# exosports/transit

Hardware: AMD Instinct MI355X
Metric: wavenumber-points*layers/sec (CH4 2-4um emission spectrum) (higher is better)
Workload: dtype f64; 1 GPU; BASELINE configs[1]: CH4-demo-shaped emission: 2500-5000 cm-1 @1 cm-1, wnosamp 2160, CH4 lines, eclipse, 5 angles, H2-H2 CIA; n_wn=2501, n_layers=100, layers_needed=81, n_lines=1000000, parallelism=one GPU

## Files before the change

transit_amd/csrc/hip/trx_api.hip:

```cpp
#include <hip/hip_runtime.h>
#include <rccl/rccl.h>
#include <dlfcn.h>

#include <algorithm>
#include <chrono>
#include <cmath>
#include <cstdio>
#include <cstdlib>
#include <cstring>
#include <atomic>
#include <condition_variable>
#include <initializer_list>
#include <memory>
#include <mutex>
#include <string>
#include <thread>
#include <vector>

#include "transit_hip.h"
#include "trx_kernels.hip.h"
#include "trx_walk.hip.h"
#include "trx_rows.hip.h"
#include "trx_tail.hip.h"
#include "trx_lanes.hip.h"
// ... 33 lines not shown
#include "../trx_launch.h"
#include "../trx_hpdata.h"

using namespace trx;

#include "trx_handle.hip.h"

namespace {

void read_switches(Switches &w)
{
  auto set = [](const char *name) { return std::getenv(name) != nullptr; };
  auto num = [](const char *name, long long otherwise) { const char *e = std::getenv(name); return e ? std::atoll(e) : otherwise; };
  auto clamped = [&](const char *name, int lo, int hi, int otherwise) { return (int)std::max<long long>(lo, std::min<long long>(hi, num(name, otherwise))); };
  w.no_row_copy = set("TRX_NO_ROW_COPY");
  w.no_rows32 = set("TRX_NO_ROWS32");
  w.row_staging = !set("TRX_NO_ROW_STAGING");
  w.row_m8_from = num("TRX_ROWS_M8_FROM", w.row_m8_from);
  w.packed_walk = !set("TRX_NO_PACKED_WALK");
  w.packed_max_layers = clamped("TRX_PACKED_MAX_LAYERS", 1, 32, w.packed_max_layers);
  w.xcd_map = (int)num("TRX_XCD_MAP", w.xcd_map);
  w.no_binrec = set("TRX_NO_BINREC");
  const long long lanes = num("TRX_LANES_WALK", 1);
  w.lanes_walk = lanes != 0; w.lanes_force = lanes == 2;
  w.lanes_parts_most = clamped("TRX_LANES_PARTS", 2, 4, w.lanes_parts_most);
  w.ray_tail = num("TRX_RAY_TAIL", 1) != 0;
  w.cia_sums = num("TRX_CIA_SUMS", 1) != 0;
  w.cia_segments = num("TRX_CIA_SEGMENTS", 1) != 0;
  w.cia_window = num("TRX_CIA_WINDOW", 1) != 0;
  w.two_queues = num("TRX_TWO_QUEUES", 1) != 0;
  w.tail_direct = num("TRX_TAIL_DIRECT", 1) != 0;
  w.range_reach = num("TRX_RANGE_REACH", 1) != 0;
  w.shard_frames = num("TRX_SHARD_FRAMES", 1) != 0;
}

struct TableBuild { TablePlan P; DevBuf d_jobs; };

template <class F>
void for_job_batches(const std::vector<ProfileJob> &jobs, F fn)
{
  for (size_t j0 = 0; j0 < jobs.size(); j0 += 32768) fn(j0, (int)std::min<size_t>(32768, jobs.size() - j0));
}

int plan_into_handle(trx_handle *h, const trx_static *s, TableBuild &B)
{
  const char *text = "";
  const TablePlanError pe = plan_table(*s, B.P, &text);
  if (pe != kTablePlanOk) return fail(h, pe == kTablePlanArg ? TRX_E_ARG : TRX_E_UNSUPPORTED, text);
  h->adop = B.P.adop; h->alor = B.P.alor; h->psize = B.P.psize; h->poff = B.P.poff; h->tab_n = B.P.tab_n;
  h->psizeT = std::move(B.P.psizeT); h->psize_mono = B.P.psize_mono;
  if (!index_steps(h->adop.data(), s->ndop, h->dopthr)) return fail(h, TRX_E_ARG, "Doppler-width grid is not strictly increasing");
  if (!index_steps(h->alor.data(), s->nlor, h->lorthr)) h->lorthr.clear();
  return TRX_OK;
}

int upload_table_inputs(trx_handle *h, const trx_static *s, TableBuild &B)
{
  int rc;
  double coef[64]; long double fact = 1.0L;
  for (int n = 0; n < 64; n++) { if (n > 0) fact *= (long double)n; coef[n] = (double)(1.0L / (fact * (long double)(2 * n + 1))); }
  HIPCHK(h, hipMemcpyToSymbolAsync(HIP_SYMBOL(c_voigt_coef), coef, sizeof(coef), 0, hipMemcpyHostToDevice, h->stream));
  if ((rc = upload(h, B.d_jobs, B.P.jobs))) return rc;
  const size_t tab_alloc = table_alloc_floats(h->tab_n, s->osamp);
  if ((rc = ensure(h, h->d_tab, sizeof(float) * tab_alloc))) return rc;
  HIPCHK(h, hipMemsetAsync(h->d_tab.p, 0, sizeof(float) * tab_alloc, h->stream));
  h->tab = h->d_tab.as<float>() + kTabPad;
// ... 514 lines not shown

struct LayerHost {
  size_t nli = 0, extra_off = 0;
  std::vector<double> &f64; std::vector<int32_t> &i32;
  const int32_t *psmax = nullptr;
  LayerHost(std::vector<double> &f, std::vector<int32_t> &i) : f64(f), i32(i) {}
};

inline double layer_negct(double temp) { return -kExpCte * kTliEfct / temp; }
inline double layer_strength(const trx_handle *h, int i, double z) { return kSigCte * h->iso_ratio[i] / (h->iso_mass[i] * z); }

inline int dop_index(const trx_handle *h, double v, int from)
{
  const double *thr = h->dopthr.data();
  while (from + 1 < h->ndop && v >= thr[from + 1]) from++;
  while (v < thr[from]) from--;
  return from;
}
inline int lor_index(const trx_handle *h, double v, int from)
{
  if (h->lorthr.empty()) return nearest_index(h->alor.data(), v, 0, h->nlor);
  const double *thr = h->lorthr.data();
  while (from + 1 < h->nlor && v >= thr[from + 1]) from++;
  while (v < thr[from]) from--;
  return from;
}
inline int dop_index_far(const trx_handle *h, double v)
{
  const double *thr = h->dopthr.data();
  return (int)(std::upper_bound(thr + 1, thr + h->ndop, v) - thr) - 1;
}

int prep_layers(trx_handle *h, int nr, const double *temp_k, const double *density ,
                const double *zpart , size_t extra_doubles, LayerHost &LH)
{
  const int niso = h->niso, nmol = h->nmol;
  const size_t nli = (size_t)nr * std::max(niso, 1);
  LH.nli = nli; LH.extra_off = 7 * nli;
  LH.f64.assign(7 * nli + extra_doubles, 0.0);
  LH.i32.assign(4 * nli, 0);
  double *negct = &LH.f64[0], *strength = negct + nr, *dens = strength + nli, *alphad = dens + nli,
         *alphal = alphad + nli, *wcut = alphal + nli;
  int32_t *idop0 = &LH.i32[0], *ilor = idop0 + nli, *psmax = ilor + nli, *npre = psmax + nli;
  LH.psmax = psmax;
  h->dens_over_m.resize(nmol);
  double *dm = h->dens_over_m.data();
  h->guess_dop.assign((size_t)std::max(niso, 1), 0); h->guess_lor.assign((size_t)std::max(niso, 1), 0);
  h->guess_a0.assign((size_t)std::max(niso, 1), 0); h->guess_a1.assign((size_t)std::max(niso, 1), 0); h->guess_npre.assign((size_t)std::max(niso, 1), -1);
  for (int r = 0; r < nr; r++) {
    const double temp = temp_k[r];
    if (!(temp > 0)) return fail(h, TRX_E_ARG, "non-positive layer temperature");
    negct[r] = layer_negct(temp);
    const double fdoppler = std::sqrt(2 * kKb * temp / kAmu) * kSqrtLn2 / kLs;
    const double florentz = std::sqrt(2 * kKb * temp / kPi / kAmu) / (kAmu * kLs);
    for (int j = 0; j < nmol; j++) dm[j] = density[(size_t)j * nr + r] / h->mol_mass[j];
    for (int i = 0; i < niso; i++) {
      double al = 0.0;
      const double *csd_i = &h->pair_csd[(size_t)i * nmol], *sq_i = &h->pair_sqrt[(size_t)i * nmol];
      for (int j = 0; j < nmol; j++)
        al += dm[j] * csd_i[j] * csd_i[j] * sq_i[j];
      al *= florentz;
      const double ad = fdoppler / h->iso_sqrtm[i];
      const size_t k = (size_t)r * niso + i;
      alphal[k] = al; alphad[k] = ad;
      idop0[k] = h->guess_dop[i] = dop_index(h, ad * h->wn_i, h->guess_dop[i]);
      ilor[k]  = h->guess_lor[i] = lor_index(h, al, h->guess_lor[i]);
      strength[k] = layer_strength(h, i, zpart[(size_t)i * nr + r]);
      dens[k] = density[(size_t)h->iso_imol[i] * nr + r];
      wcut[k] = doppler_refresh_cut(ad, al);
      const bool has_lines = h->iso_wmax[i] > 0;
      const int a0 = has_lines ? (h->guess_a0[i] = dop_index(h, ad * h->iso_wmin[i], h->guess_a0[i])) : idop0[k];
      const int a1 = has_lines ? (h->guess_a1[i] = dop_index(h, ad * h->iso_wmax[i], h->guess_a1[i])) : idop0[k];
      const int32_t *psl = &h->psizeT[(size_t)ilor[k] * h->ndop];
      auto widest_of = [&](int i0, int i1) {
        if (i0 > i1) std::swap(i0, i1);
        if (h->psize_mono) return psl[i1];
        int32_t m = 0;
        for (int d = i0; d <= i1; d++) m = std::max(m, psl[d]);
        return m;
      };
      int32_t pm = widest_of(std::min(idop0[k], std::min(a0, a1)), std::max(idop0[k], std::max(a0, a1)));
      if (h->sw.shard_frames && has_lines) {
// ... 441 lines not shown
}

static int run_check(trx_handle *h, const trx_atm *a, const trx_opts *o)
{
  const int nr = a->nlayer;
  if (nr < 3) return fail(h, TRX_E_ARG, "at least three layers are needed");
  if (!h->saved.empty() && (int)h->saved.size() != nr) return fail(h, TRX_E_ARG, "restored extinction has another number of layers");
  if (!h->saved.empty() && h->has_grid) return fail(h, TRX_E_UNSUPPORTED, "restored extinction together with an opacity grid");
  if (o->solution != TRX_SOL_ECLIPSE && o->solution != TRX_SOL_TRANSIT) return fail(h, TRX_E_ARG, "unknown solution");
  if (o->solution == TRX_SOL_ECLIPSE && (o->nangles < 1 || o->nangles > kMaxAngles || !o->angles_deg))
    return fail(h, TRX_E_ARG, "eclipse needs 1..16 angles");
  if (o->solution == TRX_SOL_TRANSIT && o->modlevel != 1 && o->modlevel != -1) return fail(h, TRX_E_UNSUPPORTED, "modlevel must be 1 or -1");
  if (!(o->ethresh > 0)) return fail(h, TRX_E_ARG, "ethresh must be positive");
  if ((o->cloud_flag >= 2 || o->scat_flag == 2) && !a->abund && o->cloud_flag >= 2) return fail(h, TRX_E_ARG, "cloud model needs abundances");
  for (int i = 1; i < nr; i++) if (!(a->radius[i] > a->radius[i-1])) return fail(h, TRX_E_ARG, "radii must ascend");
  return TRX_OK;
}

namespace {

constexpr ScheduleCaps kScheduleCaps{kEmisRowsAbove, kTailRays, kTailSteps, 65536, kMaxChunk, kTauH};
static_assert(kTailSteps == 2, "the side-queue tail waits for ev_walk1 alone: the main queue may carry exactly one walk ahead of it");

struct Run {
  trx_handle *const h; const trx_atm *const a; const trx_opts *const o;
  double *const spectrum; void *const d_spectrum; trx_debug *const dbg; const Products want;
  const std::chrono::steady_clock::time_point t_host0;

  const int nr = a->nlayer; const int64_t nsh = h->nsh; const hipStream_t st = h->stream;
  const bool eager = o->eager != 0, prof = o->profile != 0, count = o->profile >= 2;
  const bool vertical = o->solution == TRX_SOL_ECLIPSE, extras_on = o->scat_flag != 0 || o->cloud_flag != 0;
  const bool pipelined = !h->has_grid;
  const bool stop_at_hint_ok = !h->has_grid && !eager && h->hint_layers > 0 && h->hint_layers <= nr;
  const bool stage_spec = spectrum && !d_spectrum && nsh <= (1 << 20);

  LayerHost LH{h->run_f64, h->run_i32};
  int gstride = 0; size_t mw_doubles = 0, n_geom_all = 0, nli = 0, n_f64 = 0, n_geom = 0, n_ip = 0, n_cd = 0, n_i32 = 0;
  size_t off_geom = 0, off_ip = 0, off_cd = 0, off_i32 = 0, in_bytes = 0;

  const bool ride_along = nsh <= 65536;
  bool early_front = false; double *kmax_run = nullptr; RunInit RI{};

  LayerDev Y{}; const double *d_wcut = nullptr; const int32_t *d_npre = nullptr;
  const double *d_press = nullptr, *d_tempk = nullptr, *d_mdens = nullptr, *d_nH = nullptr, *d_scatpol = nullptr, *d_rad = nullptr;
  const double *d_gw = nullptr, *d_gh0 = nullptr, *d_mw = nullptr, *d_mh0 = nullptr, *d_pw = nullptr, *d_ipv = nullptr, *d_ciadens = nullptr;
  double *d_out = nullptr; PlanInput P{};

  hipStream_t tst = nullptr;
  hipStream_t queue(Queue q) const { return q == kQMain ? st : q == kQSide ? h->stream4 : h->stream2; }
  hipEvent_t event(const QueueOp &op) const {
    switch (op.ev) {
      case kEvInputs: return h->ev_inputs; case kEvCia: return h->ev_cia; case kEvJoin: return h->ev_join; case kEvWalk1: return h->ev_walk1;
      case kEvStepDone: return h->ev_ac[(size_t)op.idx]; case kEvRecordsFree: return h->ev_cb[(size_t)op.idx];
      default: return nullptr;
    }
  }

  TailChoice tail;
  TailArgs TA{}; int tail_nct = 0;
  const size_t tail_blocks = (size_t)((nsh + kTailRays - 1) / kTailRays);

  int r_top = nr - 1; bool resumed = false;
  ScheduleState sched;
  CombineArgs comb[2];
  std::vector<uint8_t> layer_walked;

  int flags[8] = {}, status[4] = {}; double ms_cia = 0;
  std::vector<unsigned long long> counters;
  Spans spans; Spans *const sp = prof ? &spans : nullptr;
  std::chrono::steady_clock::time_point t_host_prep = t_host0, t_host_queued = t_host0, t_lap = t_host0;
  const bool lap_on = log_sink().fn && log_sink().max_level >= TRX_LOG_DEBUG; std::string laps;

  bool in_flight = false;
  ~Run() { if (in_flight) { (void)hipStreamSynchronize(h->stream4); (void)hipStreamSynchronize(h->stream2); (void)hipStreamSynchronize(h->stream); } }

  void lap(const char *what) {
    if (!lap_on) return;
    const auto n = std::chrono::steady_clock::now();
    char b[64]; std::snprintf(b, sizeof b, " %s %.0f", what, 1e3 * std::chrono::duration<double, std::milli>(n - t_lap).count());
    laps += b; t_lap = n;
  }
  void model_args(TauArgs &T) const; void tau_args(TauArgs &T, int r_top_, int nc_) const; void emis_args(EmisArgs &E) const; void mod_args(ModArgs &M) const;
  void launch_tau(const TauArgs &T, hipStream_t q) const; void launch_ray_tail() const;
  void launch_run_init() const
  { hipLaunchKernelGGL(k_run_init, dim3((unsigned)std::min<long long>((std::max<long long>(nsh, 3LL * nr) + 255) / 256, 65536)), dim3(256), 0, st, RI); }
  int layout(); int front_maxima(); void host_inputs();
  int workspaces(); int front_inputs(); int grid_weights();
  int plan_first_pass(); int pass(); int resume(); int finish();
  int issue(const QueueOp &op); SweepMode sweep_mode(const QueueOp &op) const;
  int walk(const QueueOp &op); int grid_step(const PlanStep &s); int cia_group(); int restore_rows(const QueueOp &op); int tau_substep(const QueueOp &op);
  int spectrum_kernel(); int ray_tail();
  int results(const PassEnd &end);
  int product_kernels();
};

void Run::model_args(TauArgs &T) const
{
  T.nr = nr; T.nsh = nsh; T.lo = h->lo; T.wn_i = h->wn_i; T.wn_d = h->wn_d; T.wn_fct = o->wn_fct;
  T.scat_flag = o->scat_flag; T.cloud_flag = o->cloud_flag; T.nmol = h->nmol;
  T.scat_pref = std::pow(10.0, o->scat_logext) * kE0H2;
  T.press = d_press; T.temp = d_tempk; T.scat_pol = d_scatpol;
  T.cloud_top = o->cloud_top; T.cloud_bot = o->cloud_bot; T.cloud_ext = o->cloud_ext; T.cloud_gamma = o->cloud_gamma;
  T.cloud_Q = o->cloud_Q; T.cloud_r = o->cloud_r; T.cloud_sig = o->cloud_sig; T.cloud_refwn = o->cloud_refwn;
  T.mdens = d_mdens; T.nH = d_nH;
  if (extras_on) { T.xf_scat = h->d_xf.as<double>(); T.xf_cloud = T.xf_scat + nsh; T.xf_const = T.xf_cloud + nsh; }
}

void Run::tau_args(TauArgs &T, int r_top_, int nc_) const
{
  T.solution = o->solution; T.rad_fct = a->rad_fct; T.toomuch = o->toomuch;
  T.r_top = r_top_; T.nc = nc_; T.rad = d_rad; T.e = h->d_e.as<double>(); T.ecs = h->d_ecs.as<double>();
  T.er = h->d_er.as<double>(); T.tau = h->d_tau.as<double>(); T.last = h->d_last.as<int>();
  T.er_all = (dbg != nullptr || eager) ? 1 : 0;
  T.gw = d_gw; T.gstride = gstride; T.gh0 = d_gh0;
  model_args(T);
  T.flags = h->d_flags.as<int>(); T.eager = eager;
  T.pw = d_pw; T.acc = h->d_acc.as<double>(); T.lay = vertical ? d_pw + 6 * (size_t)nr : nullptr;
  T.hrs = d_pw + 4 * (size_t)nr; T.hr0 = T.hrs + nr; T.status = h->d_status.as<int>();
}

void Run::emis_args(EmisArgs &E) const
// ... 50 lines not shown
  n_f64 = 7 * nli + 8 * (size_t)nr; n_geom = vertical ? n_geom_all : 1; n_ip = (size_t)nr; n_cd = (size_t)nr * h->cia.size(); n_i32 = 4 * nli;
  off_geom = n_f64; off_ip = off_geom + n_geom; off_cd = off_ip + n_ip; off_i32 = off_cd + n_cd;
  in_bytes = (8 * off_i32 + 4 * n_i32 + 8 + 15) & ~(size_t)15;
  if ((rc = ensure_pinned(h, h->h_in, in_bytes)) || (rc = ensure(h, h->d_in, in_bytes)) || (rc = ensure_small(h, nr)) ||
      (rc = ensure(h, h->d_last, sizeof(int) * nsh)) || (rc = ensure(h, h->d_acc, sizeof(double) * 2 * nsh)) ||
      (rc = ensure(h, h->d_sticky, sizeof(int) * nli)))
    return rc;
  const size_t had = h->d_kmax.bytes;
  if ((rc = ensure(h, h->d_kmax, sizeof(double) * 2 * (size_t)nr))) return rc;
  if (h->d_kmax.bytes != had || !h->kmax_clean || h->kmax_nr != nr) {
    HIPCHK(h, hipMemsetAsync(h->d_kmax.p, 0, sizeof(double) * 2 * (size_t)nr, st));
    h->kmax_parity = 0; h->kmax_nr = nr;
  }
  h->kmax_clean = false;
  kmax_run = h->d_kmax.as<double>() + (size_t)h->kmax_parity * nr;
  RI.last = h->d_last.as<int>(); RI.nsh = nsh; RI.acc = h->d_acc.as<double>();
  RI.counters = h->d_counters.as<unsigned long long>(); RI.ncounters = 3 * nr;
  RI.kmax = h->d_kmax.as<double>() + (size_t)(h->kmax_parity ^ 1) * nr; RI.nkmax = nr;
  RI.status = h->d_status.as<int>(); RI.flags = h->d_flags.as<int>(); RI.rays = (int)std::min<int64_t>(nsh, 0x7fffffff);
  h->kmax_parity ^= 1;
  counters.assign(3 * (size_t)nr, 0); layer_walked.assign((size_t)nr, 0);
  in_flight = true;
  return TRX_OK;
}

int Run::front_maxima()
{
  int rc;
  early_front = !h->has_grid && h->ngroups > 0 && h->h_in.dev != nullptr;
  if (early_front) {
    double *hin = (double *)h->h_in.p;
    for (int r = 0; r < nr; r++) {
      if (!(a->temp[r] > 0)) return fail(h, TRX_E_ARG, "non-positive layer temperature");
      hin[r] = layer_negct(a->temp[r]);
      for (int i = 0; i < h->niso; i++) hin[(size_t)nr + (size_t)r * h->niso + i] = layer_strength(h, i, a->zpart[(size_t)i * nr + r]);
    }
    if (!ride_along) launch_run_init();
    LayerDev Yp{}; Yp.negc_over_t = (const double *)h->h_in.dev; Yp.strength_f = Yp.negc_over_t + nr;
    bool rode = false;
    if ((rc = launch_layer_max(h, Yp, nr, a->temp, 1, nullptr, st, kmax_run, ride_along ? &RI : nullptr, &rode))) return rc;
    lap("max");
  }
  if ((rc = prep_layers(h, nr, a->temp, a->density, a->zpart, 8 * (size_t)nr, LH))) return rc;
  lap("layers");
  h->walk_temp_ok = true;
  for (int r = 0; r < nr; r++) if (a->temp[r] < kWalkMinTemp) h->walk_temp_ok = false;
  host_inputs();
  lap("rays");
  if (LH.f64.size() != n_f64 || h->run_geom.size() != n_geom || h->run_ipv.size() != n_ip || LH.i32.size() != n_i32)
    return fail(h, TRX_E_HIP, "internal: the input block's layout");
  return TRX_OK;
}

void Run::host_inputs()
{
  const int nmol = h->nmol;
  std::vector<double> &f64 = LH.f64, &geom = h->run_geom, &ipv = h->run_ipv;
  double *press = &f64[LH.extra_off], *tempk = press + nr, *mdens = tempk + nr, *nH = mdens + nr,
         *scat_pol = nH + nr, *radv = scat_pol + nr;
  for (int r = 0; r < nr; r++) {
    press[r] = a->press ? a->press[r] : 0.0; tempk[r] = a->temp[r]; radv[r] = a->radius[r];
    double mm = 0, md = 0, sp = 0;
    for (int j = 0; j < nmol; j++) {
      const double d = a->density[(size_t)j * nr + r];
      if (a->abund) {
        const double q = a->abund[(size_t)j * nr + r];
        md += d / h->mol_mass[j] * q;
        if (h->mol_is_h2[j]) nH[r] = d / h->mol_mass[j] * q * kNavo;
        mm += h->mol_mass[j] * q;
      }
      sp += kPi * 8e-32 / 3. * std::pow(h->mol_pol[j], 2) * d / h->mol_mass[j] * kNavo;
    }
    mdens[r] = md * mm; scat_pol[r] = sp;
  }

  geom.assign(vertical ? n_geom_all : 1, 0.0);
  if (vertical) {
    std::vector<double> sx(nr + 1);
    double *gw = &geom[0], *gh0 = gw + (size_t)(nr + 1) * gstride;
    double *pw = gh0 + (nr + 1) + mw_doubles + (nr + 1);
    const int rs = nr - 2;
    const double r3[3] = {a->radius[rs], (a->radius[rs] + a->radius[rs+1]) / 2.0, a->radius[rs+1]};
    sx[0] = 0.0;
    for (int i = 1; i < 3; i++) sx[i] = sx[i-1] + (r3[i] - r3[i-1]);
    simpson_weights(sx.data(), 3, gw + (size_t)rs * gstride, gh0 + rs);
    for (int k = 0; k + 2 < nr; k++) { double h0; simpson_weights(a->radius + k, 3, pw + 4 * (size_t)k, &h0); }
    double *lay = pw + 6 * (size_t)nr;
    for (int rs = 0; rs < nr; rs++) {
      double *L = lay + (size_t)kVertLay * rs;
      if (rs + 1 < nr) {
        const double step = a->radius[rs + 1] - a->radius[rs];
        L[0] = step; L[1] = a->radius[rs] / step; L[2] = 2.0 * step * step;
        L[8] = 1.0 / step; L[9] = 1.0 / L[2]; L[10] = L[1] + 1.5;
      }
      for (int q = 0; q < 4; q++) L[3 + q] = pw[4 * (size_t)rs + q];
      L[7] = a->radius[rs]; L[11] = a->radius[rs] * a->radius[rs];
    }
  }
  ipv.resize((size_t)nr);
  for (int i = 0; i < nr; i++) ipv[i] = a->radius[nr - 1 - i];
}

int Run::workspaces()
{
  int rc;
  const int user_chunk = o->layer_chunk > 0 ? std::max(3, o->layer_chunk) : 0;
  h->run_frame.resize((size_t)nr); h->run_wide.resize((size_t)nr);
  const bool any_wide = layer_frames(h, LH.psmax, nr, h->run_frame.data(), h->run_wide.data());
  const size_t gr_b = (size_t)std::max<int64_t>(h->ngroups, 1);
  P.sg_layers = any_wide ? (user_chunk ? std::min(user_chunk, kMaxChunk) : kMaxChunk) : 1;
  P.frame = h->run_frame.data(); P.very_wide = h->run_wide.data(); P.nr = nr; P.hint_layers = h->hint_layers; P.user_chunk = user_chunk;
  P.eager = eager; P.has_grid = h->has_grid; P.stop_at_hint_ok = stop_at_hint_ok; P.walk_cap = kWalkLayers; P.chunk_cap = kMaxChunk;
  if ((rc = ensure(h, h->d_SG, sizeof(double) * gr_b * P.sg_layers)) || (rc = ensure(h, h->d_idop8, gr_b * P.sg_layers)) ||
      (rc = ensure(h, h->d_e, sizeof(double) * nr * nsh)) || (rc = ensure(h, h->d_er, sizeof(double) * nr * nsh)) ||
      (rc = ensure(h, h->d_tau, sizeof(double) * nr * nsh)) ||
      (rc = ensure(h, h->d_intens, sizeof(double) * kMaxAngles * nsh)) || (rc = ensure(h, h->d_spec, sizeof(double) * nsh)))
    return rc;
  if (pipelined)
    while ((int)h->ev_ac.size() < nr + 1) {
      hipEvent_t e1, e2;
      if (hipEventCreateWithFlags(&e1, hipEventDisableTiming) != hipSuccess ||
          hipEventCreateWithFlags(&e2, hipEventDisableTiming) != hipSuccess) return fail(h, TRX_E_HIP, "event");
      h->ev_ac.push_back(e1); h->ev_cb.push_back(e2);
    }
  if (count && any_wide && (rc = ensure(h, h->d_part3, 24 * (size_t)kMaxChunk * ((((size_t)((nsh + kTileBins - 1) / kTileBins) + 3) / 4) + kXcds * kAccumXcdGroup))))
    return rc;
  return ensure(h, h->d_ecs, sizeof(double) * (size_t)nr * nsh);
}

int Run::front_inputs()
{
  int rc;
  double *hin = (double *)h->h_in.p;
  const size_t skip = early_front ? (size_t)nr + nli : 0;
  std::memcpy(hin + skip, LH.f64.data() + skip, 8 * (n_f64 - skip));
  std::memcpy(hin + off_geom, h->run_geom.data(), 8 * n_geom);
  std::memcpy(hin + off_ip, h->run_ipv.data(), 8 * n_ip);
  cia_densities(h, a, hin + off_cd);
  std::memcpy(hin + off_i32, LH.i32.data(), 4 * n_i32);
  lap("block");
  t_host_prep = std::chrono::steady_clock::now();
  lap("prep");
  if (!early_front) { HIPCHK(h, hipMemcpyAsync(h->d_in.p, h->h_in.p, in_bytes, hipMemcpyHostToDevice, st)); lap("h2d"); }
  if (dbg || eager || (h->ngroups == 0 && !h->has_grid)) HIPCHK(h, hipMemsetAsync(h->d_e.p, 0, sizeof(double) * nr * nsh, st));
  if (dbg || eager) HIPCHK(h, hipMemsetAsync(h->d_tau.p, 0, sizeof(double) * nr * nsh, st));

  const double *df = h->d_in.as<double>();
  layer_dev(df, (const int32_t *)(df + off_i32), LH, nr, Y, d_wcut, d_npre);
  d_press = df + LH.extra_off; d_tempk = d_press + nr; d_mdens = d_tempk + nr; d_nH = d_mdens + nr; d_scatpol = d_nH + nr; d_rad = d_scatpol + nr;
  if (!vertical && (rc = ensure(h, h->d_geom, sizeof(double) * n_geom_all))) return rc;
  d_gw = vertical ? df + off_geom : h->d_geom.as<double>(); d_gh0 = d_gw + (size_t)(nr + 1) * gstride;
  d_mw = d_gh0 + (nr + 1); d_mh0 = d_mw + mw_doubles; d_pw = d_mh0 + (nr + 1);
  d_ipv = df + off_ip; d_ciadens = df + off_cd;
  if (h->has_grid && (rc = grid_weights())) return rc;
  if (early_front) {
    const double *pf = (const double *)h->h_in.dev;
    LayerDev Yp{}; const double *p_wcut; const int32_t *p_npre;
    layer_dev(pf, (const int32_t *)(pf + off_i32), LH, nr, Yp, p_wcut, p_npre);
    if ((rc = launch_sticky(h, Yp, p_npre, nr, 1, nullptr, o->ethresh, st, kmax_run, pf, h->d_in.p, in_bytes))) return rc;
  } else {
    if (!ride_along) launch_run_init();
    bool rode = false;
    if (!h->has_grid &&
        (rc = layer_maxima_and_sticky(h, Y, d_npre, nr, a->temp, 1, nullptr, o->ethresh, st, kmax_run, ride_along ? &RI : nullptr, &rode))) return rc;
    if (ride_along && !rode) launch_run_init();
  }
  HIPCHK(h, hipEventRecord(h->ev_inputs, st));
  lap("kmax");
  return extras_on ? ensure(h, h->d_xf, sizeof(double) * (2 * (size_t)nsh + 8)) : TRX_OK;
}

int Run::grid_weights()
{
  if (h->og_nlayer != nr) return fail(h, TRX_E_ARG, "opacity grid has a different number of layers");
  const int nt = (int)h->og_ntemp, nm = (int)h->og_nmol;
  std::vector<double> &og_layer = h->run_og_layer; std::vector<int> &og_itemp = h->run_og_itemp;
  og_layer.assign((size_t)(3 + nm) * nr, 0.0); og_itemp.assign((size_t)nr, 0);
  for (int r = 0; r < nr; r++) {
    const double temp = a->temp[r];
    if (temp < h->og_temp[0] || !(temp < h->og_temp[nt - 1])) return fail(h, TRX_E_RANGE, "layer temperature outside the opacity grid");
    int it = nearest_index(h->og_temp.data(), temp, 0, nt);
    if (temp < h->og_temp[it]) it--;
    og_itemp[r] = it;
    og_layer[r] = h->og_temp[it + 1] - temp; og_layer[nr + r] = temp - h->og_temp[it];
    og_layer[2 * (size_t)nr + r] = h->og_temp[it + 1] - h->og_temp[it];
    for (int m = 0; m < nm; m++) og_layer[(size_t)(3 + m) * nr + r] = a->density[(size_t)h->og_molidx[m] * nr + r];
  }
  const int rc = upload(h, h->d_og_layer, og_layer);
  return rc ? rc : upload(h, h->d_og_itemp, og_itemp);
}


int Run::plan_first_pass()
{
  int rc;
  if (!h->ev_run_a) { HIPCHK(h, hipEventCreate(&h->ev_run_a)); HIPCHK(h, hipEventCreate(&h->ev_run_b)); }
  if (prof) HIPCHK(h, hipEventRecord(h->ev_run_a, st));
  h->stats.walk_steps = 0; h->stats.walk_records = 0; h->stats.walk_record_lanes = 0;
  for (int k = 0; k < 3; k++) h->stats.walk_form_steps[k] = h->stats.walk_form_layers[k] = h->stats.walk_form_record_lanes[k] = 0;
  if (!h->has_grid && lap_on) {
    std::string ln = "run: walk frame (bins) per layer, top first; 0 = two-kernel form:";
    for (int r = nr - 1; r >= 0; r--) ln += " " + std::to_string(h->run_frame[r]);
    log_msg(TRX_LOG_DEBUG, ln);
  }
  d_out = d_spectrum ? (double *)d_spectrum : h->d_spec.as<double>();
  plan_pass(P, r_top, stop_at_hint_ok, h->run_plan);
  TailIn ti;
  ti.ray_tail = h->sw.ray_tail; ti.tail_direct = h->sw.tail_direct; ti.two_queues = h->sw.two_queues;
  ti.stop_at_hint_ok = stop_at_hint_ok; ti.count = count; ti.has_lines = h->ngroups > 0; ti.no_saved = h->saved.empty(); ti.pipelined = pipelined;
  ti.nsh = nsh; ti.nwn = h->nwn; ti.pass = &h->run_plan;
  ti.host_spectrum = spectrum && !d_spectrum; ti.any_product = want.bs || want.px || want.br;
  tail = tail_choice(ti, kScheduleCaps);
  if ((tail.tail_spec || stage_spec) && (rc = ensure_pinned(h, h->h_spec, sizeof(double) * (size_t)nsh))) return rc;
  return tail.tail_direct ? ensure_pinned(h, h->h_tailblk, 8 * tail_blocks + 16) : TRX_OK;
}

int Run::cia_group()
{
  const auto t0 = std::chrono::steady_clock::now();
  if (extras_on) {
    TauArgs X{};
    model_args(X);
    hipLaunchKernelGGL(k_extras_factors, dim3((unsigned)((nsh + 255) / 256)), dim3(256), 0, h->stream2, X,
                       h->d_xf.as<double>(), h->d_xf.as<double>() + nsh, h->d_xf.as<double>() + 2 * nsh);
  }
  if (!vertical) {
    SlantGeomArgs G{};
    G.rad = d_rad; G.nr = nr; G.fct = a->rad_fct; G.gstride = gstride;
    G.gw = const_cast<double *>(d_gw); G.gh0 = const_cast<double *>(d_gh0); G.mw = const_cast<double *>(d_mw); G.mh0 = const_cast<double *>(d_mh0);
    G.hrs = const_cast<double *>(d_pw) + 4 * (size_t)nr; G.hr0 = G.hrs + nr;
    hipLaunchKernelGGL(k_slant_geometry, dim3((unsigned)(nr + nr - 2)), dim3(64), 0, h->stream2, G);
  }
  if (const int rcc = cia_device(h, a, o, d_tempk, d_ciadens, h->stream2)) return rcc;
  ms_cia = std::chrono::duration<double, std::milli>(std::chrono::steady_clock::now() - t0).count();
  return TRX_OK;
}

int Run::restore_rows(const QueueOp &op)
{
// ... 138 lines not shown
  t_host_queued = std::chrono::steady_clock::now();
  if (end.sync_side) HIPCHK(h, hipStreamSynchronize(h->stream4));
  HIPCHK(h, hipStreamSynchronize(st));
  if (spectrum && (tail_spec || stage_spec)) std::memcpy(spectrum, h->h_spec.p, sizeof(double) * (size_t)nsh);
  if (tail_direct) {
    const int32_t *tb = (const int32_t *)h->h_tailblk.p;
    int still = 0, deep = 0;
    for (size_t b = 0; b < tail_blocks; b++) { still += tb[2 * b]; deep = std::max(deep, tb[2 * b + 1]); }
    const int f[8] = {still, 0, tail_nct, 0, deep, 0, 0, 0};
    std::memcpy(h->h_small.p, f, sizeof f);
    int st4[4] = {0, 0, 0, 0};
    for (int code = 1; code < 4; code++) if (tb[2 * tail_blocks + code]) st4[0] = code;
    std::memcpy((char *)h->h_small.p + 64, st4, 16);
  }
  std::memcpy(flags, h->h_small.p, sizeof(flags));
  std::memcpy(status, (const char *)h->h_small.p + 64, sizeof(status));
  if (count) std::memcpy(counters.data(), (const char *)h->h_small.p + 128, 24 * (size_t)nr);
  return TRX_OK;
}

int Run::pass()
{
  int rc;
  ScheduleIn in;
  in.pipelined = pipelined; in.has_grid = h->has_grid; in.vertical = vertical; in.has_lines = h->ngroups > 0;
  in.tail = tail; in.saved = h->saved.empty() ? nullptr : h->saved.data(); in.nr = nr;
  const PassEnd end = schedule_pass(h->run_plan, in, kScheduleCaps, sched, h->run_sched);
  tst = queue(end.spectrum_q);
  for (const QueueOp &op : h->run_sched) if ((rc = issue(op))) return rc;
  r_top = h->run_plan.back().r_top - h->run_plan.back().nc;
  return (rc = product_kernels()) ? rc : results(end);
}

int Run::resume()
{
  if (tail.tail_direct) HIPCHK(h, hipMemcpyAsync(h->d_flags.p, h->h_small.p, 32, hipMemcpyHostToDevice, st));
  tail = TailChoice{};
  resumed = true; h->hint_layers = P.hint_layers = 0;
  plan_pass(P, r_top, false, h->run_plan);
  return pass();
}

int Run::finish()
{
  int rc;
  trx_stats &S = h->stats;
  S.layers_swept = flags[2];
  h->hint_layers = flags[4];
  S.neval = S.nskip = S.sum_bins = S.sum_bins_walk = S.walk_layers = 0;
  S.walk_form_bins[0] = S.walk_form_bins[1] = S.walk_form_bins[2] = 0;
  for (int r = 0; r < nr; r++) {
    S.sum_bins += (int64_t)counters[3*r]; S.neval += (int64_t)counters[3*r+1]; S.nskip += (int64_t)counters[3*r+2];
    if (const int fw = layer_walked[(size_t)r]) { S.walk_layers++; S.sum_bins_walk += (int64_t)counters[3*r]; S.walk_form_bins[fw - 1] += (int64_t)counters[3*r]; }
  }
  float ms = 0; if (prof) (void)hipEventElapsedTime(&ms, h->ev_run_a, h->ev_run_b); S.ms_run_total = ms;
  S.ms_cia = ms_cia;
  S.ms_host_total = std::chrono::duration<double, std::milli>(std::chrono::steady_clock::now() - t_host0).count();
  if (lap_on) {
    char b[160];
    std::snprintf(b, sizeof b, "run: host %.0f us preparing inputs, %.0f us queueing, %.0f us waiting for the device",
                  1e3 * std::chrono::duration<double, std::milli>(t_host_prep - t_host0).count(),
                  1e3 * std::chrono::duration<double, std::milli>(t_host_queued - t_host_prep).count(),
                  1e3 * (S.ms_host_total - std::chrono::duration<double, std::milli>(t_host_queued - t_host0).count()));
    log_msg(TRX_LOG_DEBUG, std::string(b) + "; queueing by phase (us):" + laps);
  }
  S.ms_k_sweep = S.ms_k_walk = S.ms_k_accum = S.ms_tau = S.ms_sweep = 0; S.sweep_launches = 0;
  S.ms_k_walk_form[0] = S.ms_k_walk_form[1] = S.ms_k_walk_form[2] = 0; S.ms_walk_span = 0;
  if (prof) {
    double t[Spans::kKinds] = {0, 0, 0, 0, 0, 0};
    spans.sum(t);
    S.ms_k_walk_form[0] = t[Spans::kWalk]; S.ms_k_walk_form[1] = t[Spans::kWalkLanes]; S.ms_k_walk_form[2] = t[Spans::kWalkPacked];
    S.ms_k_sweep = t[Spans::kSweep]; S.ms_k_walk = t[Spans::kWalk] + t[Spans::kWalkLanes] + t[Spans::kWalkPacked]; S.ms_k_accum = t[Spans::kAccum]; S.ms_tau = t[Spans::kTau];
    S.sweep_launches = sched.steps;
    S.ms_sweep = S.ms_k_sweep + S.ms_k_walk + S.ms_k_accum;
    S.ms_walk_span = spans.walk_span();
  }

  if (dbg) {
    if (dbg->e)    HIPCHK(h, hipMemcpy(dbg->e, h->d_e.p, sizeof(double) * nr * nsh, hipMemcpyDeviceToHost));
    if (dbg->e_cs) HIPCHK(h, hipMemcpy(dbg->e_cs, h->d_ecs.p, sizeof(double) * nr * nsh, hipMemcpyDeviceToHost));
    if (dbg->tau) {
      std::vector<double> t((size_t)nr * nsh);
      HIPCHK(h, hipMemcpy(t.data(), h->d_tau.p, sizeof(double) * nr * nsh, hipMemcpyDeviceToHost));
      for (int64_t w = 0; w < nsh; w++) for (int i = 0; i < nr; i++) dbg->tau[(size_t)w * nr + i] = t[(size_t)i * nsh + w];
    }
    if (dbg->last) {
      std::vector<int> l(nsh);
      HIPCHK(h, hipMemcpy(l.data(), h->d_last.p, sizeof(int) * nsh, hipMemcpyDeviceToHost));
      for (int64_t w = 0; w < nsh; w++) dbg->last[w] = l[w];
    }
    if (dbg->intens && o->solution == TRX_SOL_ECLIPSE)
      HIPCHK(h, hipMemcpy(dbg->intens, h->d_intens.p, sizeof(double) * o->nangles * nsh, hipMemcpyDeviceToHost));
    if (dbg->computed) for (int r = 0; r < nr; r++) dbg->computed[r] = (r >= nr - S.layers_swept) ? 1 : 0;
    if (dbg->er) HIPCHK(h, hipMemcpy(dbg->er, h->d_er.p, sizeof(double) * nr * nsh, hipMemcpyDeviceToHost));
    if (dbg->e_scat || dbg->e_cloud) {
      DevBuf d_x;
      if ((rc = ensure(h, d_x, sizeof(double) * 2 * (size_t)nr * nsh))) return rc;
// ... 103 lines not shown
```

transit_amd/csrc/hip/trx_api_sweep.hip.h:

```cpp
#pragma once

struct Spans {
  enum Kind { kSweep = 0, kWalk = 1, kAccum = 2, kTau = 3, kWalkLanes = 4, kWalkPacked = 5, kKinds = 6 };
  struct Span { hipEvent_t a, b; int kind; };
  std::vector<Span> v;
  int begin(int kind, hipStream_t st) {
    Span sp{nullptr, nullptr, kind};
    if (hipEventCreate(&sp.a) != hipSuccess || hipEventCreate(&sp.b) != hipSuccess) return -1;
    v.push_back(sp);
    return hipEventRecord(sp.a, st) == hipSuccess ? 0 : -1;
  }
  int end(hipStream_t st) { return hipEventRecord(v.back().b, st) == hipSuccess ? 0 : -1; }
  void sum(double out[kKinds]) const {
    for (const Span &sp : v) { float t = 0; if (hipEventElapsedTime(&t, sp.a, sp.b) == hipSuccess) out[sp.kind] += t; }
  }
  static bool is_walk(int k) { return k == kWalk || k == kWalkLanes || k == kWalkPacked; }
  double walk_span() const {
    double best = 0;
    for (const Span &x : v) if (is_walk(x.kind))
      for (const Span &y : v) if (is_walk(y.kind)) { float t = 0; if (hipEventElapsedTime(&t, x.a, y.b) == hipSuccess && t > best) best = t; }
    return best;
  }
  ~Spans() { for (Span &sp : v) { if (sp.a) (void)hipEventDestroy(sp.a); if (sp.b) (void)hipEventDestroy(sp.b); } }
};
// ... 248 lines not shown
  const int niso = h->niso, r_top = s.r_top, nc = s.nc;
  const int ntiles = (int)((h->nsh + kTileBins - 1) / kTileBins);
  const GroupView G = group_view(h);
  SweepWindow Wn{};
  Wn.windowed = h->windowed() ? 1 : 0; Wn.osamp = h->osamp; Wn.lo = h->lo; Wn.hi = h->hi; Wn.nwn = h->nwn;
  const long long seg_lines = sweep_window_lines(G, psmax, r_top, nc);
  constexpr unsigned kSpan = kXcds * kAccumXcdGroup;
  const unsigned tblocks = (unsigned)(((ntiles + 3) / 4 + kSpan - 1) / kSpan * kSpan);
  if (sp && sp->begin(Spans::kSweep, st)) return fail(h, TRX_E_HIP, "event");
  if (seg_lines > 0) {
    hipLaunchKernelGGL(k_group_sweep, dim3((unsigned)((seg_lines + 255) / 256)), dim3(256), sizeof(long long) * (2 * (size_t)niso + 1), st,
                       h->L, Y, Wn, niso, r_top, nc, h->d_dopthr.as<double>(), h->ndop, h->d_e2tab.as<double>(), d_wcut,
                       h->d_SG.as<double>(), h->d_idop8.as<uint8_t>(), h->d_flags.as<int>(), (int)M.eager);
  }
  if (sp && (sp->end(st) || sp->begin(Spans::kAccum, st))) return fail(h, TRX_E_HIP, "event");
  if (h->ngroups > 0) {
    AccumArgs A = accum_args(h, Y, s, M, ntiles, tblocks);
    const WideMasks K = wide_masks(G, psmax, r_top, nc, h->sw.row_m8_from);
    A.skip_mask = K.wide;
    if (M.prof) HIPCHK(h, hipMemsetAsync(h->d_part3.p, 0, 24 * (size_t)nc_max * tblocks, st));
    if (!K.all_wide) hipLaunchKernelGGL(k_accumulate, dim3(tblocks, (unsigned)nc), dim3(256), 0, st, A);
    if (K.wide) launch_wide(h, A, K, M.prof, st);
  }
  if (sp && sp->end(st)) return fail(h, TRX_E_HIP, "event");
  if (M.prof && h->ngroups > 0) {
    for (int k = 0; k < 3; k++)
      hipLaunchKernelGGL(k_sum_parts_gated, dim3((unsigned)nc), dim3(256), 0, st, h->d_part3.as<unsigned long long>(),
                         (int)tblocks, 3, k, h->d_counters.as<unsigned long long>(), 3, r_top, h->d_flags.as<int>(), (int)M.eager);
  }
  return TRX_OK;
}

int launch_layer_max(trx_handle *h, const LayerDev &Y, int nv, const double *temp_k, int nmx, const int32_t *d_iso_mx,
                     hipStream_t st, double *kmax, const RunInit *init = nullptr, bool *init_done = nullptr)
{
  if (init_done) *init_done = false;
  if (h->ngroups == 0) return TRX_OK;
  bool pruned = h->ncand > 0;
  for (int r = 0; r < nv && pruned; r++) if (kExpCte * kTliEfct * h->wn_i / temp_k[r] < 1e-5) pruned = false;
  const long long n = pruned ? h->ncand : h->nlines;
  for (int r0 = 0; r0 < nv; r0 += 32768) {
    const int nr = std::min(32768, nv - r0);
    LayerDev Yr = Y; Yr.negc_over_t += r0; Yr.strength_f += (size_t)r0 * h->niso;
    const unsigned ny = (unsigned)((nr + kLayerMaxGroup - 1) / kLayerMaxGroup);
    const bool with_init = init && r0 == 0;
    RunInit R{}; R.nsh = -1;
    if (with_init) { R = *init; *init_done = true; }
    const int xwaves = (int)std::min<long long>((n + 64 * kLayerMaxLines - 1) / (64 * kLayerMaxLines), kLayerMaxWaves);
    hipLaunchKernelGGL(k_layer_max, dim3((unsigned)((xwaves + kLayerMaxBlock - 1) / kLayerMaxBlock), ny + (with_init ? 1u : 0u)), dim3(64 * kLayerMaxBlock), sizeof(double) * (size_t)kLayerMaxGroup * (size_t)std::max(h->niso, 1), st,
                       h->L, Yr, h->niso, nr, pruned ? h->d_candrec.as<CandLine>() : nullptr, n, h->d_e2tab.as<double>(), nmx, d_iso_mx,
                       (unsigned long long *)(kmax + (size_t)r0 * nmx), R, with_init ? (int)ny : -1, xwaves);
  }
  return TRX_OK;
}

int launch_sticky(trx_handle *h, const LayerDev &Y, const int32_t *d_npre, int nv, int nmx, const int32_t *d_iso_mx, double ethresh,
                  hipStream_t st, const double *kmax, const void *copy_src = nullptr, void *copy_dst = nullptr, size_t copy_bytes = 0)
{
  const long long n16 = (long long)(copy_bytes / 16);
  if (h->ngroups == 0 && n16 == 0) return TRX_OK;
  bool copied = n16 == 0;
  for (int r0 = 0; r0 < nv || !copied; r0 += 4096) {
    const int nr = h->ngroups == 0 ? 0 : std::max(0, std::min(4096, nv - r0));
    const int nst = nr * h->niso;
    const int ncp = copied ? 0 : (int)std::min<long long>((n16 + 63) / 64, 64);
    if (nst + ncp == 0) break;
    hipLaunchKernelGGL(k_sticky_index, dim3((unsigned)(nst + ncp)), dim3(64), 0, st,
                       h->L, Y, h->niso, r0 + nr - 1, nr, kmax, nmx, d_iso_mx, ethresh, h->d_dopthr.as<double>(), h->ndop,
                       h->d_e2tab.as<double>(), d_npre, h->d_sticky.as<int>(), h->d_flags.as<int>(), 1,
                       copied ? nullptr : (const uint4 *)copy_src, copied ? nullptr : (uint4 *)copy_dst, copied ? 0LL : n16, nst);
    copied = true;
  }
  HIPCHK(h, hipGetLastError());
  return TRX_OK;
}

int layer_maxima_and_sticky(trx_handle *h, const LayerDev &Y, const int32_t *d_npre, int nv, const double *temp_k,
                            int nmx, const int32_t *d_iso_mx, double ethresh, hipStream_t st, double *kmax,
                            const RunInit *init = nullptr, bool *init_done = nullptr)
{
  int rc;
  if (init_done) *init_done = false;
  if ((rc = ensure(h, h->d_sticky, sizeof(int) * (size_t)nv * std::max(h->niso, 1)))) return rc;
  if (h->ngroups == 0) return TRX_OK;
  if ((rc = launch_layer_max(h, Y, nv, temp_k, nmx, d_iso_mx, st, kmax, init, init_done))) return rc;
  return launch_sticky(h, Y, d_npre, nv, nmx, d_iso_mx, ethresh, st, kmax);
}
```

transit_amd/csrc/hip/trx_handle.hip.h:

```cpp
#pragma once

namespace {

struct DevBuf {
  void *p = nullptr; size_t bytes = 0;
  ~DevBuf() { release(); }
  void release() { if (p) { (void)hipFree(p); p = nullptr; bytes = 0; } }
  template <class T> T *as() const { return (T *)p; }
};

struct PinnedBuf {
  void *p = nullptr, *dev = nullptr; size_t bytes = 0;
  ~PinnedBuf() { release(); }
  void release() { if (p) { (void)hipHostFree(p); p = dev = nullptr; bytes = 0; } }
};

struct DevView {
  void *p = nullptr;
  template <class T> T *as() const { return (T *)p; }
};

struct BandSet {
  int32_t nbands = 0; int64_t npieces = 0;
  DevBuf d_bands, d_pieces, d_w, d_part;
// ... 25 lines not shown
  int32_t nexp = 0;
  std::vector<double> scale, smear;
};
struct PixelRun {
  const PixelSet *set; int32_t nshift; const ObservedSet *obs = nullptr; const FilterSet *filt = nullptr; bool trail = false; PixelExtents ext{};
  const HighPassSet *hp = nullptr; HighpassExtents hpx{};
  const ExposureSet *ex = nullptr; bool ex_rows = false;
};
struct Broadening { double beta = 0, limb = 0; int hmax = 0; };
struct Products {
  const BandSet *bs = nullptr;
  bool contrib = false;
  const PixelRun *px = nullptr;
  const Broadening *br = nullptr;
};

struct Switches {
  bool no_row_copy = false;
  bool no_rows32 = false;
  bool row_staging = true;
  long long row_m8_from = 768;
  bool packed_walk = true; int packed_max_layers = 10;
  int xcd_map = 1;
  bool no_binrec = false;
  bool lanes_walk = true, lanes_force = false;
  int lanes_parts_most = 4;
  bool ray_tail = true;
  bool cia_sums = true;
  bool cia_segments = true;
  bool cia_window = true;
  bool two_queues = true;
  bool tail_direct = true;
  bool range_reach = true;
  bool shard_frames = true;
};

}

struct trx_handle {
  int device = 0;
  hipStream_t stream = nullptr, stream2 = nullptr;
  hipStream_t stream4 = nullptr;
  std::vector<hipEvent_t> ev_ac, ev_cb;
  hipEvent_t ev_walk1 = nullptr;
  hipEvent_t ev_inputs = nullptr, ev_cia = nullptr, ev_join = nullptr, ev_run_a = nullptr, ev_run_b = nullptr;
  std::string err;

  double wn_i = 0, wn_d = 0, odwn = 0; int64_t nwn = 0, nown = 0, lo = 0, hi = 0, nsh = 0; int osamp = 1;
  int niso = 0, nmol = 0;
  std::vector<double> iso_mass, iso_ratio, mol_mass, mol_radius, mol_pol;
  std::vector<double> pair_csd, pair_sqrt;
  std::vector<int32_t> iso_imol, mol_is_h2;
  std::vector<double> iso_wmin, iso_wmax;
  int ndop = 0, nlor = 0;
  std::vector<double> adop, alor;
  std::vector<int32_t> psizeT; bool psize_mono = false;
  std::vector<double> dopthr;
  std::vector<double> lorthr;
  std::vector<int> guess_dop, guess_lor, guess_a0, guess_a1;
  std::vector<long> guess_npre;
  std::vector<double> iso_sqrtm;
  std::vector<double> dens_over_m;
  std::vector<int32_t> psize; std::vector<long long> poff; int64_t tab_n = 0;
  DevBuf d_adop, d_dopthr, d_e2tab, d_psize, d_poff, d_tab, d_tabT, d_poffT, d_gimod, d_gidiv;
  float *tab = nullptr; const float *tabT = nullptr; const long long *poffT = nullptr;
  DevBuf d_tabW, d_walkprof; const float *tabW = nullptr; bool tabw_ok = false;
// ... 150 lines not shown
```

Baseline: 888.2 million wavenumber-points*layers/s.

## Prepare only the hinted top layers up front and defer the rest to resume

When a layer-count hint allows stopping early, host layer prep, the per-layer maxima kernel and the sticky-index kernel now cover only the top hinted layers (at least 3). The remaining layers are prepared, uploaded and indexed lazily in resume(), and only if the pass has to continue deeper. This is meant to remove host and GPU front-end work for layers the eclipse walk never reaches (81 of 100 needed here). In exchange it adds a second upload and kernel round if resume happens, plus a guard that fails if the plan reaches below the prepared layers.

```diff
diff --git a/transit_amd/csrc/hip/trx_api.hip b/transit_amd/csrc/hip/trx_api.hip
--- a/transit_amd/csrc/hip/trx_api.hip
+++ b/transit_amd/csrc/hip/trx_api.hip
@@ -89,6 +89,7 @@
   w.tail_direct = num("TRX_TAIL_DIRECT", 1) != 0;
   w.range_reach = num("TRX_RANGE_REACH", 1) != 0;
   w.shard_frames = num("TRX_SHARD_FRAMES", 1) != 0;
+  w.hint_front = num("TRX_HINT_FRONT", 1) != 0;
 }
 
 struct TableBuild { TablePlan P; DevBuf d_jobs; };
@@ -669,7 +670,7 @@
 }
 
 int prep_layers(trx_handle *h, int nr, const double *temp_k, const double *density ,
-                const double *zpart , size_t extra_doubles, LayerHost &LH)
+                const double *zpart , size_t extra_doubles, LayerHost &LH, int r_from = 0)
 {
   const int niso = h->niso, nmol = h->nmol;
   const size_t nli = (size_t)nr * std::max(niso, 1);
@@ -684,7 +685,8 @@
   double *dm = h->dens_over_m.data();
   h->guess_dop.assign((size_t)std::max(niso, 1), 0); h->guess_lor.assign((size_t)std::max(niso, 1), 0);
   h->guess_a0.assign((size_t)std::max(niso, 1), 0); h->guess_a1.assign((size_t)std::max(niso, 1), 0); h->guess_npre.assign((size_t)std::max(niso, 1), -1);
-  for (int r = 0; r < nr; r++) {
+  for (int r = 0; r < r_from; r++) if (!(temp_k[r] > 0)) return fail(h, TRX_E_ARG, "non-positive layer temperature");
+  for (int r = r_from; r < nr; r++) {
     const double temp = temp_k[r];
     if (!(temp > 0)) return fail(h, TRX_E_ARG, "non-positive layer temperature");
     negct[r] = layer_negct(temp);
@@ -1192,6 +1194,10 @@
   const bool vertical = o->solution == TRX_SOL_ECLIPSE, extras_on = o->scat_flag != 0 || o->cloud_flag != 0;
   const bool pipelined = !h->has_grid;
   const bool stop_at_hint_ok = !h->has_grid && !eager && h->hint_layers > 0 && h->hint_layers <= nr;
+  int r_prep = h->sw.hint_front && stop_at_hint_ok && !dbg && !count && !want.contrib && h->saved.empty()
+                 ? std::max(0, nr - std::max(h->hint_layers, 3)) : 0;
+  bool any_wide = false;
+  bool frames_logged = false;
   const bool stage_spec = spectrum && !d_spectrum && nsh <= (1 << 20);
 
   LayerHost LH{h->run_f64, h->run_i32};
@@ -1246,7 +1252,8 @@
   { hipLaunchKernelGGL(k_run_init, dim3((unsigned)std::min<long long>((std::max<long long>(nsh, 3LL * nr) + 255) / 256, 65536)), dim3(256), 0, st, RI); }
   int layout(); int front_maxima(); void host_inputs();
   int workspaces(); int front_inputs(); int grid_weights();
-  int plan_first_pass(); int pass(); int resume(); int finish();
+  int frames(); void fill_block(size_t skip); void log_frames();
+  int plan_first_pass(); int pass(); int prepare_rest(); int resume(); int finish();
   int issue(const QueueOp &op); SweepMode sweep_mode(const QueueOp &op) const;
   int walk(const QueueOp &op); int grid_step(const PlanStep &s); int cia_group(); int restore_rows(const QueueOp &op); int tau_substep(const QueueOp &op);
   int spectrum_kernel(); int ray_tail();
@@ -1363,16 +1370,17 @@
     double *hin = (double *)h->h_in.p;
     for (int r = 0; r < nr; r++) {
       if (!(a->temp[r] > 0)) return fail(h, TRX_E_ARG, "non-positive layer temperature");
+      if (r < r_prep) continue;
       hin[r] = layer_negct(a->temp[r]);
       for (int i = 0; i < h->niso; i++) hin[(size_t)nr + (size_t)r * h->niso + i] = layer_strength(h, i, a->zpart[(size_t)i * nr + r]);
     }
     if (!ride_along) launch_run_init();
     LayerDev Yp{}; Yp.negc_over_t = (const double *)h->h_in.dev; Yp.strength_f = Yp.negc_over_t + nr;
     bool rode = false;
-    if ((rc = launch_layer_max(h, Yp, nr, a->temp, 1, nullptr, st, kmax_run, ride_along ? &RI : nullptr, &rode))) return rc;
+    if ((rc = launch_layer_max(h, Yp, nr, a->temp, 1, nullptr, st, kmax_run, ride_along ? &RI : nullptr, &rode, r_prep))) return rc;
     lap("max");
   }
-  if ((rc = prep_layers(h, nr, a->temp, a->density, a->zpart, 8 * (size_t)nr, LH))) return rc;
+  if ((rc = prep_layers(h, nr, a->temp, a->density, a->zpart, 8 * (size_t)nr, LH, r_prep))) return rc;
   lap("layers");
   h->walk_temp_ok = true;
   for (int r = 0; r < nr; r++) if (a->temp[r] < kWalkMinTemp) h->walk_temp_ok = false;
@@ -1391,6 +1399,7 @@
          *scat_pol = nH + nr, *radv = scat_pol + nr;
   for (int r = 0; r < nr; r++) {
     press[r] = a->press ? a->press[r] : 0.0; tempk[r] = a->temp[r]; radv[r] = a->radius[r];
+    if (r < r_prep) continue;
     double mm = 0, md = 0, sp = 0;
     for (int j = 0; j < nmol; j++) {
       const double d = a->density[(size_t)j * nr + r];
@@ -1415,9 +1424,9 @@
     sx[0] = 0.0;
     for (int i = 1; i < 3; i++) sx[i] = sx[i-1] + (r3[i] - r3[i-1]);
     simpson_weights(sx.data(), 3, gw + (size_t)rs * gstride, gh0 + rs);
-    for (int k = 0; k + 2 < nr; k++) { double h0; simpson_weights(a->radius + k, 3, pw + 4 * (size_t)k, &h0); }
+    for (int k = r_prep; k + 2 < nr; k++) { double h0; simpson_weights(a->radius + k, 3, pw + 4 * (size_t)k, &h0); }
     double *lay = pw + 6 * (size_t)nr;
-    for (int rs = 0; rs < nr; rs++) {
+    for (int rs = r_prep; rs < nr; rs++) {
       double *L = lay + (size_t)kVertLay * rs;
       if (rs + 1 < nr) {
         const double step = a->radius[rs + 1] - a->radius[rs];
@@ -1432,17 +1441,26 @@
   for (int i = 0; i < nr; i++) ipv[i] = a->radius[nr - 1 - i];
 }
 
-int Run::workspaces()
-{
-  int rc;
-  const int user_chunk = o->layer_chunk > 0 ? std::max(3, o->layer_chunk) : 0;
+int Run::frames()
+{
+  int rc;
+  const int user_chunk = P.user_chunk;
   h->run_frame.resize((size_t)nr); h->run_wide.resize((size_t)nr);
-  const bool any_wide = layer_frames(h, LH.psmax, nr, h->run_frame.data(), h->run_wide.data());
+  any_wide = layer_frames(h, LH.psmax, nr, h->run_frame.data(), h->run_wide.data());
   const size_t gr_b = (size_t)std::max<int64_t>(h->ngroups, 1);
   P.sg_layers = any_wide ? (user_chunk ? std::min(user_chunk, kMaxChunk) : kMaxChunk) : 1;
-  P.frame = h->run_frame.data(); P.very_wide = h->run_wide.data(); P.nr = nr; P.hint_layers = h->hint_layers; P.user_chunk = user_chunk;
+  P.frame = h->run_frame.data(); P.very_wide = h->run_wide.data();
+  if ((rc = ensure(h, h->d_SG, sizeof(double) * gr_b * P.sg_layers)) || (rc = ensure(h, h->d_idop8, gr_b * P.sg_layers))) return rc;
+  return TRX_OK;
+}
+
+int Run::workspaces()
+{
+  int rc;
+  P.user_chunk = o->layer_chunk > 0 ? std::max(3, o->layer_chunk) : 0;
+  P.nr = nr; P.hint_layers = h->hint_layers;
   P.eager = eager; P.has_grid = h->has_grid; P.stop_at_hint_ok = stop_at_hint_ok; P.walk_cap = kWalkLayers; P.chunk_cap = kMaxChunk;
-  if ((rc = ensure(h, h->d_SG, sizeof(double) * gr_b * P.sg_layers)) || (rc = ensure(h, h->d_idop8, gr_b * P.sg_layers)) ||
+  if ((rc = frames()) ||
       (rc = ensure(h, h->d_e, sizeof(double) * nr * nsh)) || (rc = ensure(h, h->d_er, sizeof(double) * nr * nsh)) ||
       (rc = ensure(h, h->d_tau, sizeof(double) * nr * nsh)) ||
       (rc = ensure(h, h->d_intens, sizeof(double) * kMaxAngles * nsh)) || (rc = ensure(h, h->d_spec, sizeof(double) * nsh)))
@@ -1459,16 +1477,20 @@
   return ensure(h, h->d_ecs, sizeof(double) * (size_t)nr * nsh);
 }
 
-int Run::front_inputs()
-{
-  int rc;
+void Run::fill_block(size_t skip)
+{
   double *hin = (double *)h->h_in.p;
-  const size_t skip = early_front ? (size_t)nr + nli : 0;
   std::memcpy(hin + skip, LH.f64.data() + skip, 8 * (n_f64 - skip));
   std::memcpy(hin + off_geom, h->run_geom.data(), 8 * n_geom);
   std::memcpy(hin + off_ip, h->run_ipv.data(), 8 * n_ip);
   cia_densities(h, a, hin + off_cd);
   std::memcpy(hin + off_i32, LH.i32.data(), 4 * n_i32);
+}
+
+int Run::front_inputs()
+{
+  int rc;
+  fill_block(early_front ? (size_t)nr + nli : 0);
   lap("block");
   t_host_prep = std::chrono::steady_clock::now();
   lap("prep");
@@ -1488,12 +1510,12 @@
     const double *pf = (const double *)h->h_in.dev;
     LayerDev Yp{}; const double *p_wcut; const int32_t *p_npre;
     layer_dev(pf, (const int32_t *)(pf + off_i32), LH, nr, Yp, p_wcut, p_npre);
-    if ((rc = launch_sticky(h, Yp, p_npre, nr, 1, nullptr, o->ethresh, st, kmax_run, pf, h->d_in.p, in_bytes))) return rc;
+    if ((rc = launch_sticky(h, Yp, p_npre, nr, 1, nullptr, o->ethresh, st, kmax_run, pf, h->d_in.p, in_bytes, r_prep))) return rc;
   } else {
     if (!ride_along) launch_run_init();
     bool rode = false;
     if (!h->has_grid &&
-        (rc = layer_maxima_and_sticky(h, Y, d_npre, nr, a->temp, 1, nullptr, o->ethresh, st, kmax_run, ride_along ? &RI : nullptr, &rode))) return rc;
+        (rc = layer_maxima_and_sticky(h, Y, d_npre, nr, a->temp, 1, nullptr, o->ethresh, st, kmax_run, ride_along ? &RI : nullptr, &rode, r_prep))) return rc;
     if (ride_along && !rode) launch_run_init();
   }
   HIPCHK(h, hipEventRecord(h->ev_inputs, st));
@@ -1529,13 +1551,11 @@
   if (prof) HIPCHK(h, hipEventRecord(h->ev_run_a, st));
   h->stats.walk_steps = 0; h->stats.walk_records = 0; h->stats.walk_record_lanes = 0;
   for (int k = 0; k < 3; k++) h->stats.walk_form_steps[k] = h->stats.walk_form_layers[k] = h->stats.walk_form_record_lanes[k] = 0;
-  if (!h->has_grid && lap_on) {
-    std::string ln = "run: walk frame (bins) per layer, top first; 0 = two-kernel form:";
-    for (int r = nr - 1; r >= 0; r--) ln += " " + std::to_string(h->run_frame[r]);
-    log_msg(TRX_LOG_DEBUG, ln);
-  }
+  if (r_prep == 0) log_frames();
+  else if (lap_on) log_msg(TRX_LOG_DEBUG, "run: front end over the top " + std::to_string(nr - r_prep) + " of " + std::to_string(nr) + " layers");
   d_out = d_spectrum ? (double *)d_spectrum : h->d_spec.as<double>();
   plan_pass(P, r_top, stop_at_hint_ok, h->run_plan);
+  if (!h->run_plan.empty() && h->run_plan.back().r_top - h->run_plan.back().nc + 1 < r_prep) return fail(h, TRX_E_HIP, "internal: the plan reaches below the prepared layers");
   TailIn ti;
   ti.ray_tail = h->sw.ray_tail; ti.tail_direct = h->sw.tail_direct; ti.two_queues = h->sw.two_queues;
   ti.stop_at_hint_ok = stop_at_hint_ok; ti.count = count; ti.has_lines = h->ngroups > 0; ti.no_saved = h->saved.empty(); ti.pipelined = pipelined;
@@ -1740,8 +1760,39 @@
   return (rc = product_kernels()) ? rc : results(end);
 }
 
+void Run::log_frames()
+{
+  if (frames_logged || h->has_grid || !lap_on) return;
+  std::string ln = "run: walk frame (bins) per layer, top first; 0 = two-kernel form:";
+  for (int r = nr - 1; r >= 0; r--) ln += " " + std::to_string(h->run_frame[r]);
+  log_msg(TRX_LOG_DEBUG, ln);
+  frames_logged = true;
+}
+
+int Run::prepare_rest()
+{
+  if (r_prep == 0) return TRX_OK;
+  int rc;
+  const int r_had = r_prep;
+  r_prep = 0;
+  if ((rc = prep_layers(h, nr, a->temp, a->density, a->zpart, 8 * (size_t)nr, LH))) return rc;
+  host_inputs();
+  fill_block(0);
+  HIPCHK(h, hipMemcpyAsync(h->d_in.p, h->h_in.p, in_bytes, hipMemcpyHostToDevice, st));
+  if (!h->has_grid) {
+    if ((rc = launch_layer_max(h, Y, nr, a->temp, 1, nullptr, st, kmax_run, nullptr, nullptr, 0, r_had))) return rc;
+    if ((rc = launch_sticky(h, Y, d_npre, r_had, 1, nullptr, o->ethresh, st, kmax_run))) return rc;
+  }
+  HIPCHK(h, hipEventRecord(h->ev_inputs, st));
+  HIPCHK(h, hipStreamWaitEvent(h->stream2, h->ev_inputs, 0));
+  HIPCHK(h, hipStreamWaitEvent(h->stream4, h->ev_inputs, 0));
+  lap("rest");
+  return frames();
+}
+
 int Run::resume()
 {
+  if (const int rc = prepare_rest()) return rc;
   if (tail.tail_direct) HIPCHK(h, hipMemcpyAsync(h->d_flags.p, h->h_small.p, 32, hipMemcpyHostToDevice, st));
   tail = TailChoice{};
   resumed = true; h->hint_layers = P.hint_layers = 0;
@@ -1771,6 +1822,9 @@
                   1e3 * std::chrono::duration<double, std::milli>(t_host_queued - t_host_prep).count(),
                   1e3 * (S.ms_host_total - std::chrono::duration<double, std::milli>(t_host_queued - t_host0).count()));
     log_msg(TRX_LOG_DEBUG, std::string(b) + "; queueing by phase (us):" + laps);
+    if (r_prep > 0 && !h->has_grid && !prep_layers(h, nr, a->temp, a->density, a->zpart, 8 * (size_t)nr, LH))
+      layer_frames(h, LH.psmax, nr, h->run_frame.data(), h->run_wide.data());
+    log_frames();
   }
   S.ms_k_sweep = S.ms_k_walk = S.ms_k_accum = S.ms_tau = S.ms_sweep = 0; S.sweep_launches = 0;
   S.ms_k_walk_form[0] = S.ms_k_walk_form[1] = S.ms_k_walk_form[2] = 0; S.ms_walk_span = 0;
diff --git a/transit_amd/csrc/hip/trx_api_sweep.hip.h b/transit_amd/csrc/hip/trx_api_sweep.hip.h
--- a/transit_amd/csrc/hip/trx_api_sweep.hip.h
+++ b/transit_amd/csrc/hip/trx_api_sweep.hip.h
@@ -304,18 +304,20 @@
 }
 
 int launch_layer_max(trx_handle *h, const LayerDev &Y, int nv, const double *temp_k, int nmx, const int32_t *d_iso_mx,
-                     hipStream_t st, double *kmax, const RunInit *init = nullptr, bool *init_done = nullptr)
+                     hipStream_t st, double *kmax, const RunInit *init = nullptr, bool *init_done = nullptr,
+                     int row_from = 0, int row_to = -1)
 {
   if (init_done) *init_done = false;
   if (h->ngroups == 0) return TRX_OK;
   bool pruned = h->ncand > 0;
   for (int r = 0; r < nv && pruned; r++) if (kExpCte * kTliEfct * h->wn_i / temp_k[r] < 1e-5) pruned = false;
   const long long n = pruned ? h->ncand : h->nlines;
-  for (int r0 = 0; r0 < nv; r0 += 32768) {
-    const int nr = std::min(32768, nv - r0);
+  if (row_to < 0) row_to = nv;
+  for (int r0 = row_from; r0 < row_to; r0 += 32768) {
+    const int nr = std::min(32768, row_to - r0);
     LayerDev Yr = Y; Yr.negc_over_t += r0; Yr.strength_f += (size_t)r0 * h->niso;
     const unsigned ny = (unsigned)((nr + kLayerMaxGroup - 1) / kLayerMaxGroup);
-    const bool with_init = init && r0 == 0;
+    const bool with_init = init && r0 == row_from;
     RunInit R{}; R.nsh = -1;
     if (with_init) { R = *init; *init_done = true; }
     const int xwaves = (int)std::min<long long>((n + 64 * kLayerMaxLines - 1) / (64 * kLayerMaxLines), kLayerMaxWaves);
@@ -327,12 +329,13 @@
 }
 
 int launch_sticky(trx_handle *h, const LayerDev &Y, const int32_t *d_npre, int nv, int nmx, const int32_t *d_iso_mx, double ethresh,
-                  hipStream_t st, const double *kmax, const void *copy_src = nullptr, void *copy_dst = nullptr, size_t copy_bytes = 0)
+                  hipStream_t st, const double *kmax, const void *copy_src = nullptr, void *copy_dst = nullptr, size_t copy_bytes = 0,
+                  int row_from = 0)
 {
   const long long n16 = (long long)(copy_bytes / 16);
   if (h->ngroups == 0 && n16 == 0) return TRX_OK;
   bool copied = n16 == 0;
-  for (int r0 = 0; r0 < nv || !copied; r0 += 4096) {
+  for (int r0 = row_from; r0 < nv || !copied; r0 += 4096) {
     const int nr = h->ngroups == 0 ? 0 : std::max(0, std::min(4096, nv - r0));
     const int nst = nr * h->niso;
     const int ncp = copied ? 0 : (int)std::min<long long>((n16 + 63) / 64, 64);
@@ -349,12 +352,12 @@
 
 int layer_maxima_and_sticky(trx_handle *h, const LayerDev &Y, const int32_t *d_npre, int nv, const double *temp_k,
                             int nmx, const int32_t *d_iso_mx, double ethresh, hipStream_t st, double *kmax,
-                            const RunInit *init = nullptr, bool *init_done = nullptr)
+                            const RunInit *init = nullptr, bool *init_done = nullptr, int row_from = 0)
 {
   int rc;
   if (init_done) *init_done = false;
   if ((rc = ensure(h, h->d_sticky, sizeof(int) * (size_t)nv * std::max(h->niso, 1)))) return rc;
   if (h->ngroups == 0) return TRX_OK;
-  if ((rc = launch_layer_max(h, Y, nv, temp_k, nmx, d_iso_mx, st, kmax, init, init_done))) return rc;
-  return launch_sticky(h, Y, d_npre, nv, nmx, d_iso_mx, ethresh, st, kmax);
-}
+  if ((rc = launch_layer_max(h, Y, nv, temp_k, nmx, d_iso_mx, st, kmax, init, init_done, row_from))) return rc;
+  return launch_sticky(h, Y, d_npre, nv, nmx, d_iso_mx, ethresh, st, kmax, nullptr, nullptr, 0, row_from);
+}
diff --git a/transit_amd/csrc/hip/trx_handle.hip.h b/transit_amd/csrc/hip/trx_handle.hip.h
--- a/transit_amd/csrc/hip/trx_handle.hip.h
+++ b/transit_amd/csrc/hip/trx_handle.hip.h
@@ -81,6 +81,7 @@
   bool two_queues = true;
   bool tail_direct = true;
   bool range_reach = true;
+  bool hint_front = true;
   bool shard_frames = true;
 };
 
```

Result: slower. 854.1 million wavenumber-points*layers/s (-3.8%).
